# nemochina2008/soundgen_beta

Measured on AMD Instinct MI355X. Metric: synthesized audio samples/sec (whole node) @44.1 kHz; RMS error vs R ref, higher is better.
Workload: dtype fp32 (fp64 phase)

## Files before the change

### soundgen_beta_amd/csrc/sg_exec.cpp

```cpp
#include "sg_exec.h"
#include "sg_amp.h"
#include "sg_launch.h"
#include "sg_sine_check.h"
#include "sg_prof.h"

#include <algorithm>
#include <chrono>
#include <exception>
#include <thread>
#include <cmath>
#include <climits>
#include <atomic>
#include <map>
#include <cstdlib>
#include <cstdio>
#include <cstring>
#include <string>
#include <type_traits>

namespace sg {

static void split_finalize_tiles(Batch& B) {
  const int64_t copy_tile = SG_COPY_TILE;
  B.fin_tiles.clear();
  B.fin_tiles_hp.clear();
  B.copy_tiles.clear();
  for (const SgSylTile& t : B.syl_tiles) {
    const SgSyllable& sy = B.syls[t.syl];
    if (sy.hp) {
      B.fin_tiles_hp.push_back(t);
      continue;
    }
    const int64_t end = std::min<int64_t>(t.k0 + 1024, sy.L);
    const int pend = sy.piece0 + sy.npiece;
    bool ok = sy.env.kind == 0 && sy.drift.nk == 0 && sy.genv.kind == 0;
    for (int p = t.piece; ok && p < pend && B.pieces[p].start < end; ++p) ok = B.pieces[p].nterms <= 0;
    if (!ok) {
      B.fin_tiles.push_back(t);
      continue;
    }
    for (int p = t.piece; p < pend && B.pieces[p].start < end; ++p) {
      const SgPiece& pc = B.pieces[p];
      const int64_t a = std::max<int64_t>(t.k0, pc.start), b = std::min<int64_t>(end, pc.start + pc.len);
      if (b <= a) continue;
      SgCopyTile c{};
      const bool zero = pc.nterms == 0;
      c.src = zero ? 0 : pc.t[0].src + (a - pc.start);
      c.dst = sy.out_off + a;
      c.k0 = a;
      c.L = sy.L;
      c.n = (int32_t)(b - a);
      c.max_slot = sy.max_slot;
      c.fade = sy.fade;
      c.syl = t.syl;
      c.flags = (sy.dst_fs ? SG_COPY_FS : 0) | (zero ? SG_COPY_ZERO : 0) |
                (!zero && ((c.src - c.dst) & 3) == 0 ? SG_COPY_VEC : 0);
      if (!B.copy_tiles.empty()) {
        SgCopyTile& q = B.copy_tiles.back();
        if ((q.flags & SG_COPY_VEC) && (c.flags & SG_COPY_VEC) && q.syl == c.syl && q.flags == c.flags &&
            q.k0 + q.n == c.k0 && q.src + q.n == c.src && q.n + c.n <= copy_tile) {
          q.n += c.n;
          continue;
        }
      }
      B.copy_tiles.push_back(c);
    }
  }
}

static bool direct_on() {
  const char* e = std::getenv("SG_TAB_DIRECT");
  return !(e && e[0] == '0');
}

struct TabSpans {
  std::vector<SgTabJob> jobs;
  std::vector<uint8_t> in_tab;
  std::vector<uint8_t> direct_syl;
  int64_t tasks = 0, direct = 0;
  int64_t samples = 0, terms = 0;
};
struct ColumnReader {
  const Batch& B;
  std::vector<std::pair<int64_t, int32_t>> by_off;
  std::vector<double> lg;
  explicit ColumnReader(const Batch& b) : B(b) {
    for (size_t j = 0; j < B.ampjobs.size(); ++j) by_off.push_back({B.ampjobs[j].amp_off, (int32_t)j});
    std::sort(by_off.begin(), by_off.end());
    lg.resize((size_t)B.amp_lg_rows + 2);
    for (size_t k = 0; k < lg.size(); ++k) lg[k] = std::log2((double)(k + 1));
  }
  int logn_max = SG_TAB_LOGN_MAX;
  int logn(int64_t a_off, int32_t Rn) const {
    auto it = std::upper_bound(by_off.begin(), by_off.end(), std::make_pair(a_off, INT32_MAX));
    if (it == by_off.begin()) return 0;
    const SgAmpJob& J = B.ampjobs[(size_t)std::prev(it)->second];
    const int64_t rel = a_off - J.amp_off;
    if (J.Rp <= 0 || rel % J.Rp != 0 || rel / J.Rp >= J.G || Rn > J.Rp) return 0;
    const int g = (int)(rel / J.Rp);
    double s0 = 0, s4 = 0;
    for (int r = 0; r < Rn; ++r) {
      double a = 0;
      if (r < J.R) a = J.src_off >= 0 ? (double)B.ampsrc[(size_t)(J.src_off + (int64_t)g * J.Rp + r)]
                                      : (double)(float)amp_value(B.ampcols.data() + J.col0, J, lg.data(), g, r);
      const double k = r + 1.0;
      s0 += std::fabs(a);
      s4 += std::fabs(a) * k * k * k * k;
    }
    if (!(s0 > 0)) return 0;
    const double two_pi4 = 1558.5454565440389;
    for (int b = SG_TAB_LOGN_MIN; b <= logn_max; ++b) {
      const double n4 = std::ldexp(1.0, 4 * b);
      if (two_pi4 * s4 / (384.0 * n4) <= SG_TAB_TOL * s0) return b;
    }
    return 0;
  }
};
struct TaskBlock {
  int64_t o;
  const SgWTask* p;
  int64_t n;
};
static std::vector<TaskBlock> task_blocks(const Batch& B) {
  std::vector<TaskBlock> tb;
  bulk_each(B.tasks_x, B.tasks, [&](int64_t o, const SgWTask* p, int64_t n) { tb.push_back(TaskBlock{o, p, n}); });
  return tb;
}
template <class F>
static void for_blocks(size_t n, F&& f) {
  const size_t nt = std::min<size_t>(n, std::min(16u, std::max(1u, std::thread::hardware_concurrency())));
  if (nt <= 1) {
    for (size_t i = 0; i < n; ++i) f(i);
    return;
  }
  std::atomic<size_t> next{0};
  std::vector<std::exception_ptr> errs(nt);
  auto work = [&](size_t t) {
    try {
      for (size_t i; (i = next.fetch_add(1)) < n;) f(i);
    } catch (...) {
      errs[t] = std::current_exception();
    }
  };
  std::vector<std::thread> pool;
  for (size_t t = 1; t < nt; ++t) pool.emplace_back(work, t);
  work(0);
  for (auto& th : pool) th.join();
  for (auto& e : errs)
    if (e) std::rethrow_exception(e);
}
struct TabBlock {
  std::vector<SgTabJob> jobs;
  int64_t direct = 0, samples = 0, terms = 0;
};
static void group_block(const Batch& B, const ColumnReader& cols, const TaskBlock& blk, TabSpans& S, TabBlock& out) {
  auto tab_task = [](const SgWTask& t) {
    return t.flags == (SG_TASK_CONST | SG_TASK_LIN) && t.R <= SG_ROWS_F32 && t.Rn > 0;
  };
  auto direct_ok = [&](const SgWTask& t, int64_t r0, int64_t r1) {
    if (t.syl < 0 || t.syl >= (int32_t)B.syls.size() || !direct_on()) return false;
    const SgSyllable& sy = B.syls[(size_t)t.syl];
    if (sy.hp || sy.env.kind != 0 || sy.genv.kind != 0 || sy.drift.nk != 0 || sy.nptile != 0) return false;
    if (r0 != sy.task0 || r1 != sy.task0 + sy.ntask || r1 - r0 > SG_TAB_TASKS) return false;
    for (int32_t p = sy.piece0; p < sy.piece0 + sy.npiece; ++p)
      if (B.pieces[(size_t)p].nterms > 0) return false;
    return true;
  };
  const int per_job = SG_TAB_TASKS;
  int64_t run0 = -1, run_samples = 0;
  SgWTask first{};
  auto close_run = [&](int64_t end) {
    if (run0 < 0) return;
    const int logn = run_samples >= (int64_t(4) << SG_TAB_LOGN_MIN) ? cols.logn(first.a_off, first.Rn) : 0;
    if (logn && run_samples >= (int64_t(4) << logn)) {
      const bool dir = end - run0 <= per_job && direct_ok(first, run0, end);
      if (dir) {
        S.direct_syl[(size_t)first.syl] = 1;
        ++out.direct;
      }
      for (int64_t i = run0; i < end; i += per_job) {
        const int32_t n = (int32_t)std::min<int64_t>(per_job, end - i);
        out.jobs.push_back(SgTabJob{first.a_off, first.Rn, (int32_t)i, n, logn, first.syl, dir ? SG_TAB_DIRECT : 0});
        for (int64_t q = i; q < i + n; ++q) S.in_tab[(size_t)q] = 1;
      }
      out.samples += run_samples;
      out.terms += run_samples * first.Rn;
    }
    run0 = -1;
  };
  for (int64_t k = 0; k < blk.n; ++k) {
    const SgWTask& t = blk.p[k];
    const bool ok = tab_task(t);
    if (run0 >= 0 && !(ok && t.a_off == first.a_off && t.Rn == first.Rn && t.syl == first.syl)) close_run(blk.o + k);
    if (ok && run0 < 0) {
      run0 = blk.o + k;
      first = t;
      run_samples = 0;
    }
    if (ok) run_samples += t.len;
  }
  close_run(blk.o + blk.n);
}
struct TaskClasses {
  std::vector<int32_t> tlong, tshort, tall, tallp, thp;
  std::vector<int32_t> srun, trun;
};
static void run_start(std::vector<int32_t>& runs, const std::vector<int32_t>& list, int32_t& syl, const SgWTask& t) {
  const int32_t pos = (int32_t)list.size() - 1;
  if (runs.empty() || t.syl != syl || pos - runs.back() >= SG_RUN_TASKS) runs.push_back(pos);
  syl = t.syl;
}
static void classify_block(const TaskBlock& blk, const std::vector<uint8_t>& in_tab, TaskClasses& c) {
  int32_t ssyl = -1, tsyl = -1;
  for (int64_t k = 0; k < blk.n; ++k) {
    const SgWTask& t = blk.p[k];
    const int32_t i = (int32_t)(blk.o + k);
    const bool shrt = t.len <= 64 && !(t.flags & SG_TASK_ENV);
    if (!in_tab.empty() && in_tab[(size_t)i]) continue;
    if (t.flags & SG_TASK_HP) c.thp.push_back(i);
    else if (t.R > SG_ROWS_F32) {
      if (shrt) {
        c.tallp.push_back(i);
        run_start(c.trun, c.tallp, tsyl, t);
      } else {
        c.tall.push_back(i);
      }
    } else if (shrt) {
      c.tshort.push_back(i);
      run_start(c.srun, c.tshort, ssyl, t);
    } else {
      c.tlong.push_back(i);
    }
  }
}
static TabSpans group_tables(const Batch& B, bool tables, TaskClasses* classes) {
  TabSpans S;
  const std::vector<TaskBlock> tb = task_blocks(B);
  std::vector<TabBlock> tabs(tb.size());
  std::vector<TaskClasses> cls(classes ? tb.size() : 0);
  if (tables) {
    S.in_tab.assign((size_t)bulk_size(B.tasks_x, B.tasks), 0);
    S.direct_syl.assign(B.syls.size(), 0);
  }
  const ColumnReader cols(B);
  for_blocks(tb.size(), [&](size_t i) {
    if (tables) group_block(B, cols, tb[i], S, tabs[i]);
    if (classes) classify_block(tb[i], S.in_tab, cls[i]);
  });
  for (TabBlock& t : tabs) {
    S.jobs.insert(S.jobs.end(), t.jobs.begin(), t.jobs.end());
    S.direct += t.direct;
    S.samples += t.samples;
    S.terms += t.terms;
  }
  for (const SgTabJob& j : S.jobs) S.tasks += j.n;
  if (classes) {
    auto cat = [&](std::vector<int32_t> TaskClasses::*m) {
      std::vector<int32_t>& dst = classes->*m;
      dst.clear();
      size_t n = 0;
      for (const TaskClasses& c : cls) n += (c.*m).size();
      dst.reserve(n);
      for (const TaskClasses& c : cls) dst.insert(dst.end(), (c.*m).begin(), (c.*m).end());
    };
    auto runs = [&](std::vector<int32_t> TaskClasses::*r, std::vector<int32_t> TaskClasses::*m) {
      std::vector<int32_t>& dst = classes->*r;
      dst.clear();
      int32_t base = 0;
      for (const TaskClasses& c : cls) {
        for (int32_t x : c.*r) dst.push_back(base + x);
        base += (int32_t)(c.*m).size();
      }
      dst.push_back(base);
    };
    runs(&TaskClasses::srun, &TaskClasses::tshort);
    runs(&TaskClasses::trun, &TaskClasses::tallp);
    cat(&TaskClasses::tlong);
    cat(&TaskClasses::tshort);
    cat(&TaskClasses::tall);
    cat(&TaskClasses::tallp);
    cat(&TaskClasses::thp);
  }
  return S;
}

static void debug_plan_stats(const Batch& B) {
  std::fprintf(stderr, "sg plan: %zu sine tasks, %zu syllables, %zu copy tiles, %zu general finalize tiles\n",
               (size_t)bulk_size(B.tasks_x, B.tasks), B.syls.size(), B.copy_tiles.size(), B.fin_tiles.size());
  {
    double fry = 0, plain = 0;
    int64_t nfry = 0;
    for (const SgEpoch& e : B.epochs) {
      const double b = (double)(2 * e.G - 1) * e.R * 4;
      if (e.invD < 1) { fry += b; ++nfry; } else plain += b;
    }
    std::fprintf(stderr, "sg plan: amplitude bytes: plain epochs %.3g, subharmonic epochs %.3g (%lld of %zu)\n", plain,
                 fry, (long long)nfry, B.epochs.size());
  }
  {
    const TabSpans T = group_tables(B, true, nullptr);
    int64_t cl = 0, cl_samples = 0;
    bulk_each(B.tasks_x, B.tasks, [&](int64_t, const SgWTask* p, int64_t n) {
      for (int64_t k = 0; k < n; ++k)
        if (p[k].flags == (SG_TASK_CONST | SG_TASK_LIN)) { ++cl; cl_samples += p[k].len; }
    });
    int64_t hist[13] = {0};
    for (const SgTabJob& j : T.jobs) ++hist[j.logn];
    std::fprintf(stderr, "sg plan: wavetable jobs %zu, %lld direct syllables (N = 256/512/1024/2048: %lld %lld %lld %lld; %zu tasks, %lld samples, %.3g terms); CONST|LIN tasks %lld (%lld samples)\n",
                 T.jobs.size(), (long long)T.direct, (long long)hist[8], (long long)hist[9], (long long)hist[10], (long long)hist[11],
                 (size_t)T.tasks, (long long)T.samples, (double)T.terms, (long long)cl,
                 (long long)cl_samples);
  }
  {
    int64_t all = 0, ident = 0, ni = 0, ident_items = 0, noisy = 0, noisy_cov = 0, other = 0, env_only = 0, env_kind[4] = {0, 0, 0, 0};
    for (const SgMix& m : B.mixes[0]) {
      all += m.len;
      bool id = m.mult.kind == 0 && m.am_lo == 0 && m.to_fs == 1 && m.base_kind == SG_BASE_NONE;
      for (int32_t i = m.item0; i < m.item0 + m.nitems && id; ++i) {
        const SgNoiseItem& it = B.items[(size_t)i];
        id = it.ola < 0 && it.fade < 2 && it.strength.kind == 0 && !(it.flags & SG_ITEM_F64);
      }
      if (id) { ident += m.len; ident_items += m.nitems; }
      ni += m.nitems;
      if (!id && m.mult.kind == 0 && m.to_fs == 1) {
        std::vector<std::pair<int64_t, int64_t>> iv;
        for (int32_t i = m.item0; i < m.item0 + m.nitems; ++i) {
          const SgNoiseItem& it = B.items[(size_t)i];
          if (it.ola >= 0) iv.push_back({std::max<int64_t>(0, it.off), std::min(m.len, it.off + it.len)});
        }
        std::sort(iv.begin(), iv.end());
        int64_t cov = 0, e = 0;
        for (auto& q : iv) { const int64_t a0 = std::max(q.first, e); if (q.second > a0) cov += q.second - a0; e = std::max(e, q.second); }
        noisy += m.len;
        noisy_cov += cov;
      } else if (!id) {
        other += m.len;
        bool vo = m.to_fs == 1;
        for (int32_t i = m.item0; i < m.item0 + m.nitems && vo; ++i) vo = B.items[(size_t)i].ola < 0;
        if (vo && m.mult.kind != 0) { env_only += m.len; env_kind[m.mult.kind & 3]++; }
      }
    }
    std::fprintf(stderr, "sg plan: pre-filter mixes %zu, %lld samples; voiced-only %lld samples (%lld of %lld items)\n",
                 B.mixes[0].size(), (long long)all, (long long)ident, (long long)ident_items, (long long)ni);
    std::fprintf(stderr, "sg plan: pre-filter mixes with noise %lld samples (%lld under noise), enveloped or fp64 %lld "
                 "(voiced-only with the global envelope %lld; contour kinds 1/2/3: %lld %lld %lld)\n",
                 (long long)noisy, (long long)noisy_cov, (long long)other, (long long)env_only, (long long)env_kind[1],
                 (long long)env_kind[2], (long long)env_kind[3]);
  }
  {
    int64_t j1 = 0, jm = 0, cols = 0, bins = 0;
    for (const SgEnvJob& j : B.envjobs) {
      (j.nc == 1 ? j1 : jm)++;
      cols += j.nc;
      bins += (int64_t)j.nc * j.nr;
    }
    std::fprintf(stderr, "sg plan: envelope jobs %zu (%lld one-column), %lld columns, %lld bins, %zu wave tasks\n",
                 B.envjobs.size(), (long long)j1, (long long)cols, (long long)bins, B.envtasks.size());
  }
  std::vector<SgWTask> tasks;
  bulk_each(B.tasks_x, B.tasks, [&](int64_t, const SgWTask* p, int64_t n) { tasks.insert(tasks.end(), p, p + n); });
  double terms[2] = {0, 0};
  int64_t ntask[2] = {0, 0}, rmax = 0, samples[2] = {0, 0};
  std::map<int, int64_t> rh;
  int64_t nshort[2] = {0, 0}, lh[2][5] = {{0}};
  double sterms[2] = {0, 0};
  {
    int64_t nh = 0, sh = 0, lh64 = 0;
    double th = 0, rn = 0;
    for (const SgWTask& t : tasks)
      if (t.flags & SG_TASK_HP) {
        ++nh; sh += t.len; lh64 += t.len <= 64;
        th += (double)t.Rn * t.len * ((t.flags & SG_TASK_CONST) ? 1 : 2);
        rn += t.Rn;
      }
    std::fprintf(stderr, "sg plan: fp64 tasks %lld (%lld samples, %lld of <= 64 samples, %.3g chain terms, mean Rn %.1f)\n",
                 (long long)nh, (long long)sh, (long long)lh64, th, nh ? rn / nh : 0.0);
  }
  for (const SgWTask& t : tasks) {
    const int k = t.R > SG_ROWS_F32 ? 1 : 0;
    terms[k] += (double)t.R * t.len * ((t.flags & SG_TASK_CONST) ? 1 : 2);
    ++ntask[k];
    samples[k] += t.len;
    if (t.len <= 64) { ++nshort[k]; sterms[k] += (double)t.R * t.len * ((t.flags & SG_TASK_CONST) ? 1 : 2); }
    lh[k][t.len <= 64 ? 0 : t.len <= 128 ? 1 : t.len <= 256 ? 2 : t.len <= 512 ? 3 : 4]++;
    if (k) {
      rmax = std::max<int64_t>(rmax, t.R);
      rh[t.R < 256 ? 0 : t.R < 512 ? 1 : t.R < 1024 ? 2 : t.R < 2048 ? 3 : 4]++;
    }
  }
  std::fprintf(stderr, "sg plan: sine tasks fp32 %lld (%lld samples, %.3g chain terms), tall %lld (%lld samples, %.3g chain terms, max R %lld; R<256 %lld, <512 %lld, <1024 %lld, <2048 %lld, more %lld)\n",
               (long long)ntask[0], (long long)samples[0], terms[0], (long long)ntask[1], (long long)samples[1], terms[1],
               (long long)rmax, (long long)rh[0], (long long)rh[1], (long long)rh[2], (long long)rh[3], (long long)rh[4]);
  for (int k = 0; k < 2; ++k)
    std::fprintf(stderr, "sg plan: %s tasks <= 64 samples: %lld (%.3g chain terms); len <=64/128/256/512/more: %lld %lld %lld %lld %lld\n",
                 k ? "tall" : "fp32", (long long)nshort[k], sterms[k], (long long)lh[k][0], (long long)lh[k][1],
                 (long long)lh[k][2], (long long)lh[k][3], (long long)lh[k][4]);
}

void finalize_plan(Batch& B) {
  split_finalize_tiles(B);
  if (std::getenv("SG_DEBUG_PLAN")) debug_plan_stats(B);
  B.ptiles.clear();
  bool any_hp = false;
  for (int pass = 0; pass < 2; ++pass) {
    if (pass == 1) B.ptile_hp = (int64_t)B.ptiles.size();
    for (size_t s = 0; s < B.syls.size(); ++s) {
      SgSyllable& sy = B.syls[s];
      if ((sy.hp != 0) != (pass == 1)) continue;
      any_hp |= sy.hp != 0;
      sy.ptile0 = (int32_t)B.ptiles.size();
      for (int32_t p = sy.piece0; p < sy.piece0 + sy.npiece; ++p)
        if (B.pieces[p].nterms > 0)
          for (int64_t q0 = 0; q0 < B.pieces[p].len; q0 += 256) B.ptiles.push_back(SgSylTile{(int32_t)s, p, q0});
      sy.nptile = (int32_t)B.ptiles.size() - sy.ptile0;
    }
  }
  B.slices.clear();
  const int64_t nsyl = (int64_t)B.syls.size();
  if (nsyl == 0) return;
  int64_t total = 0;
  for (const SgSyllable& sy : B.syls) total += sy.L;
  int slices = SG_SLICES;
  if (any_hp) slices = 1;
  const int K = (int)std::min<int64_t>(slices, nsyl);
  int64_t acc = 0, ft = 0, ct = 0;
  int32_t s0 = 0;
  for (int32_t s = 0; s < nsyl; ++s) {
    acc += B.syls[s].L;
    const bool cut = s == nsyl - 1 || acc * K >= total * ((int64_t)B.slices.size() + 1);
    if (!cut) continue;
    Slice c{};
    c.s0 = s0; c.s1 = s + 1;
    c.t0 = B.syls[s0].task0;
    c.t1 = B.syls[s].task0 + B.syls[s].ntask;
    c.p0 = K == 1 ? 0 : B.syls[s0].ptile0;
    c.p1 = K == 1 ? B.ptile_hp : B.syls[s].ptile0 + B.syls[s].nptile;
    c.f0 = ft;
    while (ft < (int64_t)B.fin_tiles.size() && B.fin_tiles[ft].syl <= s) ++ft;
    c.f1 = ft;
    c.c0 = ct;
    while (ct < (int64_t)B.copy_tiles.size() && B.copy_tiles[ct].syl <= s) ++ct;
    c.c1 = ct;
    B.slices.push_back(c);
    s0 = s + 1;
  }
}

int64_t device_bytes(const Batch& B) { return (int64_t)arena_bytes(arena_counts(B)); }

void device_free(DevicePlan& D) {
  if (D.arena) (void)hipFree(D.arena);
  if (D.tabbuf) (void)hipFree(D.tabbuf);
  D.pcm.free();
// ... 384 lines not shown
```

### soundgen_beta_amd/csrc/sg_harm.hip

```cpp
#include <hip/hip_runtime.h>

#include "sg_dev.h"

#include "sg_amp.h"
#include "sg_devfn.h"

using sgd::contour_at;
using sgd::linear_at;
using sgd::wave_max;

constexpr int SG_LDS_ROWS = 256;



template <bool TWO>
__device__ __forceinline__ void stage_rows(float* __restrict__ la, float* __restrict__ ld, const float* __restrict__ A,
                                           const float* __restrict__ A1, int r0, int n, int lane) {
  for (int r = lane; r < n; r += 64) {
    const float a = A[r0 + r];
    la[r] = a;
    if (TWO) ld[r] = A1[r0 + r] - a;
  }
}

typedef float f2 __attribute__((ext_vector_type(2)));
__device__ __forceinline__ float vfma(float a, float b, float c) { return fmaf(a, b, c); }
__device__ __forceinline__ double vfma(double a, double b, double c) { return fma(a, b, c); }
__device__ __forceinline__ f2 vfma(f2 a, f2 b, f2 c) { return __builtin_elementwise_fma(a, b, c); }

#define SG_ROW(a, d)                                                  \
  {                                                                   \
    _Pragma("unroll") for (int s = 0; s < NS; ++s) {                  \
      const Acc av = TWO ? vfma(tt[s], (Acc)(d), (Acc)(a)) : (Acc)(a); \
      const Acc b = vfma(al[s], b1[s], av - b2[s]);                   \
      b2[s] = b1[s];                                                  \
      b1[s] = b;                                                      \
    }                                                                 \
  }
constexpr int SG_ROWS_IT = 8;
template <int NS, bool TWO, typename Acc>
__device__ __forceinline__ void clenshaw_lds(const float* __restrict__ la, const float* __restrict__ ld, int n,
                                             const Acc (&al)[NS], const Acc (&tt)[NS], Acc (&b1)[NS], Acc (&b2)[NS]) {
  const float4 z4 = make_float4(0.f, 0.f, 0.f, 0.f);
  if (n & 4) {
    const float4 A4 = *reinterpret_cast<const float4*>(la + n - 4);
    const float4 D4 = TWO ? *reinterpret_cast<const float4*>(ld + n - 4) : z4;
    SG_ROW(A4.w, D4.w)
    SG_ROW(A4.z, D4.z)
    SG_ROW(A4.y, D4.y)
    SG_ROW(A4.x, D4.x)
    n -= 4;
  }
#pragma unroll 1
  for (int r = n - SG_ROWS_IT; r >= 0; r -= SG_ROWS_IT) {
    const float4 A4 = *reinterpret_cast<const float4*>(la + r + 4);
    const float4 D4 = TWO ? *reinterpret_cast<const float4*>(ld + r + 4) : z4;
    const float4 A0 = *reinterpret_cast<const float4*>(la + r);
    const float4 D0 = TWO ? *reinterpret_cast<const float4*>(ld + r) : z4;
    SG_ROW(A4.w, D4.w)
    SG_ROW(A4.z, D4.z)
    SG_ROW(A4.y, D4.y)
    SG_ROW(A4.x, D4.x)
    SG_ROW(A0.w, D0.w)
    SG_ROW(A0.z, D0.z)
    SG_ROW(A0.y, D0.y)
    SG_ROW(A0.x, D0.x)
  }
}

template <bool TWO, bool LIN>
__device__ __forceinline__ void sample_setup(const SgWTask& T, int l, float& t, float& al, float& sn) {
  t = TWO ? fmaf((float)l, T.xby, T.tc0) * T.rdx : 0.f;
  const double m = (double)(T.mbase + l);
  const double P = LIN ? fma(m, T.c1, T.c0) : fma(m, fma(m, fma(m, fma(m, T.c4, T.c3), T.c2), T.c1), T.c0);
  const double v = P;
  const float x = (float)(v - rint(v));
  sn = __builtin_amdgcn_sinf(x);
  al = 2.f * __builtin_amdgcn_cosf(x);
}

template <int NS, bool TWO>
__device__ __forceinline__ void clenshaw_pk(const float* __restrict__ la, const float* __restrict__ ld, int n,
                                            const float (&al)[NS], const float (&tt)[NS], float (&b1)[NS],
                                            float (&b2)[NS]) {
  constexpr int NP = NS / 2;
  f2 al2[NP], t2[NP], p1[NP], p2[NP];
#pragma unroll
  for (int i = 0; i < NP; ++i) {
    al2[i] = f2{al[2 * i], al[2 * i + 1]};
    t2[i] = f2{tt[2 * i], tt[2 * i + 1]};
    p1[i] = f2{b1[2 * i], b1[2 * i + 1]};
    p2[i] = f2{b2[2 * i], b2[2 * i + 1]};
  }
  clenshaw_lds<NP, TWO, f2>(la, ld, n, al2, t2, p1, p2);
#pragma unroll
  for (int i = 0; i < NP; ++i) {
    b1[2 * i] = p1[i].x; b1[2 * i + 1] = p1[i].y;
    b2[2 * i] = p2[i].x; b2[2 * i + 1] = p2[i].y;
  }
}
template <int NS, bool TWO, typename Acc>
__device__ __forceinline__ void clenshaw_any(const float* __restrict__ la, const float* __restrict__ ld, int n,
                                             const Acc (&al)[NS], const Acc (&tt)[NS], Acc (&b1)[NS], Acc (&b2)[NS]) {
  if constexpr (sizeof(Acc) == 4 && NS % 2 == 0)
    clenshaw_pk<NS, TWO>(la, ld, n, al, tt, b1, b2);
  else
    clenshaw_lds<NS, TWO, Acc>(la, ld, n, al, tt, b1, b2);
}

template <bool TWO, bool LIN>
__device__ __forceinline__ void sample_setup(const SgWTask& T, int l, float& t, double& al, double& sn) {
  t = TWO ? fmaf((float)l, T.xby, T.tc0) * T.rdx : 0.f;
  const double m = (double)(T.mbase + l);
  const double P = LIN ? fma(m, T.c1, T.c0) : fma(m, fma(m, fma(m, fma(m, T.c4, T.c3), T.c2), T.c1), T.c0);
  double cs;
  sincospi(2.0 * (P - rint(P)), &sn, &cs);
  al = 2.0 * cs;
}

template <int NS, bool TWO, bool ENV, bool LIN, typename Acc, typename WT = float>
__device__ __forceinline__ void run_slots(const SgWTask& T, bool staged, float* __restrict__ la, float* __restrict__ ld,
                                          const float* __restrict__ amps, const SgSyllable* __restrict__ syls,
                                          const double* __restrict__ cknots, WT* __restrict__ W, int l0, int lane,
                                          float& tmax, const float (&rc)[8], const float (&rs)[8]) {
  constexpr bool ROT = LIN && sizeof(Acc) == 4 && NS > 1;
  float t[NS];
  Acc al[NS], sn[NS], b1[NS], b2[NS];
  int l[NS];
  bool valid[NS];
#pragma unroll
  for (int s = 0; s < NS; ++s) {
    l[s] = l0 + 64 * s + lane;
    valid[s] = l[s] < T.len;
    b1[s] = b2[s] = (Acc)0;
    if (ROT && s > 0) {
      t[s] = TWO ? fmaf((float)l[s], T.xby, T.tc0) * T.rdx : 0.f;
      const float h = 0.5f * (float)al[0], s2 = 2.f * (float)sn[0];
      al[s] = fmaf((float)al[0], rc[s], -s2 * rs[s]);
      sn[s] = fmaf((float)sn[0], rc[s], h * rs[s]);
    } else {
      sample_setup<TWO, LIN>(T, valid[s] ? l[s] : 0, t[s], al[s], sn[s]);
    }
  }
  Acc tt[NS];
#pragma unroll
  for (int s = 0; s < NS; ++s) tt[s] = (Acc)t[s];
  if (staged) {
    clenshaw_any<NS, TWO, Acc>(la, ld, T.Rn, al, tt, b1, b2);
  } else {
    for (int r0 = (T.Rn - 1) / SG_LDS_ROWS * SG_LDS_ROWS; r0 >= 0; r0 -= SG_LDS_ROWS) {
      const int n = T.Rn - r0 < SG_LDS_ROWS ? T.Rn - r0 : SG_LDS_ROWS;
      stage_rows<TWO>(la, ld, amps + T.a_off, amps + T.d_off, r0, n, lane);
      clenshaw_any<NS, TWO, Acc>(la, ld, n, al, tt, b1, b2);
    }
  }
  const int jp0 = T.j0 + l0;
  if (!ENV && l0 + 64 * NS <= T.len && jp0 >= T.dj0 && jp0 + 64 * NS <= T.dj1) {
    WT* __restrict__ wp = W + T.w_off + jp0 + lane;
// ... 135 lines not shown
}

template <bool TWO>
__device__ __forceinline__ void run_pair(const SgWTask& P, const SgWTask& Q, float* __restrict__ la,
                                         float* __restrict__ ld, const float* __restrict__ amps,
                                         float* __restrict__ W, int lane, float& mp, float& mq,
                                         ColCache* cc = nullptr) {
#ifdef SG_DIAG_PAIR_NOROWS
  const int R = 0;
#else
  const int R = P.Rn > Q.Rn ? P.Rn : Q.Rn;
#endif
  if (SG_RUN_CACHE && cc) {
    const bool pc = P.flags & SG_TASK_CONST, qc = Q.flags & SG_TASK_CONST;
    ColCache nc;
    const int hn = (P.R > 64 || Q.R > 64) ? 2 : 1;
#pragma unroll
    for (int h = 0; h < 2; ++h) {
      if (h >= hn) break;
      const int r = lane + 64 * h;
      auto load = [&](int64_t off, int rows) { return r < rows ? amps[off + r] : 0.f; };
      const float pa = P.a_off == cc->off ? cc->v[h] : load(P.a_off, P.R);
      const float pd = TWO && !pc ? (P.d_off == cc->off ? cc->v[h] : load(P.d_off, P.R)) : pa;
      const float qa = Q.a_off == P.a_off ? pa
                       : Q.a_off == P.d_off && TWO && !pc ? pd
                       : Q.a_off == cc->off ? cc->v[h] : load(Q.a_off, Q.R);
      const float qd = TWO && !qc ? (Q.d_off == P.d_off && !pc ? pd : load(Q.d_off, Q.R)) : qa;
      if (r < R) {
        *reinterpret_cast<float2*>(la + 2 * r) = make_float2(pa, qa);
        if (TWO) *reinterpret_cast<float2*>(ld + 2 * r) = make_float2(pc ? 0.f : pd - pa, qc ? 0.f : qd - qa);
      }
      nc.v[h] = TWO && !qc ? qd : qa;
    }
    nc.off = TWO && !qc ? Q.d_off : Q.a_off;
    *cc = nc;
  } else {
    stage_pair<TWO>(P, Q, amps, la, ld, 0, R, lane);
  }
  const bool vp = lane < P.len, vq = lane < Q.len;
  float tp, alp, snp, tq, alq, snq;
  sample_setup<TWO, false>(P, vp ? lane : 0, tp, alp, snp);
  sample_setup<TWO, false>(Q, vq ? lane : 0, tq, alq, snq);
  const f2 al{alp, alq}, tpq{tp, tq};
  f2 b1{0.f, 0.f}, b2{0.f, 0.f};
#define SG_PROW(a, d)                                   \
  {                                                     \
    const f2 av = TWO ? vfma(tpq, (d), (a)) : (a);      \
    const f2 b = vfma(al, b1, av - b2);                 \
    b2 = b1;                                            \
    b1 = b;                                             \
  }
  const float4 z4 = make_float4(0.f, 0.f, 0.f, 0.f);
#pragma unroll 1
  for (int r = R - 4; r >= 0; r -= 4) {
    const float4 A1 = *reinterpret_cast<const float4*>(la + 2 * r + 4);
    const float4 A0 = *reinterpret_cast<const float4*>(la + 2 * r);
    const float4 D1 = TWO ? *reinterpret_cast<const float4*>(ld + 2 * r + 4) : z4;
    const float4 D0 = TWO ? *reinterpret_cast<const float4*>(ld + 2 * r) : z4;
    SG_PROW((f2{A1.z, A1.w}), (f2{D1.z, D1.w}))
    SG_PROW((f2{A1.x, A1.y}), (f2{D1.x, D1.y}))
    SG_PROW((f2{A0.z, A0.w}), (f2{D0.z, D0.w}))
    SG_PROW((f2{A0.x, A0.y}), (f2{D0.x, D0.y}))
  }
#undef SG_PROW
  pair_store(P, Q, b1.x * snp, b1.y * snq, W, lane, mp, mq);
}

extern "C" __global__ __launch_bounds__(256) __attribute__((amdgpu_waves_per_eu(8))) void sg_sine_bank(
    const int32_t* __restrict__ idx, int64_t n, const SgWTask* __restrict__ tasks, const float* __restrict__ amps,
    const SgSyllable* __restrict__ syls, const double* __restrict__ cknots, float* __restrict__ W,
    float* __restrict__ taskmax) {
  __shared__ __attribute__((aligned(16))) float rows[4][2][SG_LDS_ROWS];
  const int lane = threadIdx.x & 63;
  const int wave = __builtin_amdgcn_readfirstlane(threadIdx.x >> 6);
  const int64_t k = (int64_t)sgd::xcd_swizzle(blockIdx.x, gridDim.x) * 4 + wave;
  if (k >= n) return;
  const int64_t ti = idx[k];
  const SgWTask T = tasks[ti];
  const float wm = wave_max(run_one(T, rows[wave][0], rows[wave][1], amps, syls, cknots, W, lane));
  if (lane == 0) taskmax[ti] = wm;
}

template <bool IDXPF, class PAIR>
__device__ __forceinline__ void run_of_pairs(const int32_t* __restrict__ idx, const int32_t* __restrict__ rs,
                                             int64_t nruns, const SgWTask* __restrict__ tasks,
                                             float* __restrict__ taskmax, PAIR&& pair) {
  const int lane = threadIdx.x & 63;
  const int wave = __builtin_amdgcn_readfirstlane(threadIdx.x >> 6);
  const int64_t r = (int64_t)sgd::xcd_swizzle(blockIdx.x, gridDim.x) * 4 + wave;
  if (r >= nruns) return;
  const int32_t k0 = rs[r], k1 = rs[r + 1];
  float m = -INFINITY;
  int32_t ip = idx[k0], iq = idx[k0 + 1 < k1 ? k0 + 1 : k0];
  for (int32_t k = k0; k < k1; k += 2) {
    if (!IDXPF) {
      ip = idx[k];
      iq = idx[k + 1 < k1 ? k + 1 : k];
    }
    const SgWTask P = tasks[ip];
    const SgWTask Q = tasks[iq];
    if (IDXPF && k + 2 < k1) {
      ip = idx[k + 2];
      iq = idx[k + 3 < k1 ? k + 3 : k + 2];
    }
    float mp, mq;
    pair(P, Q, wave, lane, mp, mq);
    m = fmaxf(m, fmaxf(mp, mq));
    __asm__ __volatile__("" ::: "memory");
  }
  m = wave_max(m);
  for (int32_t k = k0 + lane; k < k1; k += 64) taskmax[idx[k]] = k == k0 ? m : -INFINITY;
}

extern "C" __global__ __launch_bounds__(256) void sg_sine_bank_pairs(
    const int32_t* __restrict__ idx, const int32_t* __restrict__ rs, int64_t nruns,
    const SgWTask* __restrict__ tasks, const float* __restrict__ amps, float* __restrict__ W,
    float* __restrict__ taskmax) {
  __shared__ __attribute__((aligned(16))) float rows[4][2][SG_LDS_ROWS];
  ColCache cc;
  run_of_pairs<true>(idx, rs, nruns, tasks, taskmax,
               [&](const SgWTask& P, const SgWTask& Q, int wave, int lane, float& mp, float& mq) {
                 if ((P.flags & Q.flags) & SG_TASK_CONST) run_pair<false>(P, Q, rows[wave][0], rows[wave][1], amps, W, lane, mp, mq, &cc);
                 else run_pair<true>(P, Q, rows[wave][0], rows[wave][1], amps, W, lane, mp, mq, &cc);
               });
}


__device__ __forceinline__ void rs_setup(const SgWTask& T, int l, bool two, float& t, float& u, float& sg, float& sn) {
  t = two ? fmaf((float)l, T.xby, T.tc0) * T.rdx : 0.f;
  const double m = (double)(T.mbase + l);
  const double P = fma(m, fma(m, fma(m, fma(m, T.c4, T.c3), T.c2), T.c1), T.c0);
  const float x = (float)(P - rint(P));
  const float h = 3.14159265358979f * x;
  const float h2 = h * h;
  float s = fmaf(h2, 1.6059043836821614e-10f, -2.5052108385441720e-08f);
  s = fmaf(h2, s, 2.7557319223985893e-06f);
  s = fmaf(h2, s, -1.9841269841269841e-04f);
  s = fmaf(h2, s, 8.3333333333333333e-03f);
  s = fmaf(h2, s, -1.6666666666666667e-01f);
  s = fmaf(h2 * s, h, h);
  float c = fmaf(h2, -1.1470745597729725e-11f, 2.0876756987868099e-09f);
  c = fmaf(h2, c, -2.7557319223985891e-07f);
  c = fmaf(h2, c, 2.4801587301587302e-05f);
  c = fmaf(h2, c, -1.3888888888888889e-03f);
  c = fmaf(h2, c, 4.1666666666666667e-02f);
  c = fmaf(h2, c, -0.5f);
  c = fmaf(h2, c, 1.f);
  sn = 2.f * s * c;
  const bool pos = fabsf(x) <= 0.25f;
  sg = pos ? 1.f : -1.f;
  u = pos ? -4.f * s * s : 4.f * c * c;
}

template <bool TWO>
__device__ __forceinline__ void run_pair_rs(const SgWTask& P, const SgWTask& Q, float* __restrict__ la,
                                            float* __restrict__ ld, const float* __restrict__ amps,
                                            float* __restrict__ W, int lane, float& mp, float& mq) {
  const int R = P.Rn > Q.Rn ? P.Rn : Q.Rn;
  const bool vp = lane < P.len, vq = lane < Q.len;
  float tp, up, sgp, snp, tq, uq, sgq, snq;
  rs_setup(P, vp ? lane : 0, TWO, tp, up, sgp, snp);
  rs_setup(Q, vq ? lane : 0, TWO, tq, uq, sgq, snq);
  const f2 u{up, uq}, sg{sgp, sgq}, tpq{tp, tq};
  f2 b{0.f, 0.f}, d{0.f, 0.f};
#define SG_RPROW(a, dd)                                  \
  {                                                      \
    const f2 av = TWO ? vfma(tpq, (dd), (a)) : (a);      \
    f2 q = vfma(sg, d, av);                              \
    q = vfma(u, b, q);                                   \
    b = vfma(sg, b, q);                                  \
    d = q;                                               \
  }
  const float4 z4 = make_float4(0.f, 0.f, 0.f, 0.f);
  constexpr int CH = SG_LDS_ROWS / 2;
#pragma unroll 1
  for (int r0 = (R - 1) / CH * CH; r0 >= 0; r0 -= CH) {
    const int n = R - r0 < CH ? R - r0 : CH;
    stage_pair<TWO>(P, Q, amps, la, ld, r0, n, lane);
#pragma unroll 1
    for (int r = n - 4; r >= 0; r -= 4) {
      const float4 A1 = *reinterpret_cast<const float4*>(la + 2 * r + 4);
      const float4 A0 = *reinterpret_cast<const float4*>(la + 2 * r);
      const float4 D1 = TWO ? *reinterpret_cast<const float4*>(ld + 2 * r + 4) : z4;
      const float4 D0 = TWO ? *reinterpret_cast<const float4*>(ld + 2 * r) : z4;
      SG_RPROW((f2{A1.z, A1.w}), (f2{D1.z, D1.w}))
      SG_RPROW((f2{A1.x, A1.y}), (f2{D1.x, D1.y}))
      SG_RPROW((f2{A0.z, A0.w}), (f2{D0.z, D0.w}))
      SG_RPROW((f2{A0.x, A0.y}), (f2{D0.x, D0.y}))
    }
  }
#undef SG_RPROW
  pair_store(P, Q, b.x * snp, b.y * snq, W, lane, mp, mq);
}

__device__ __forceinline__ float run_one_tall(const SgWTask& T, float* __restrict__ la, float* __restrict__ ld,
                                              const float* __restrict__ amps, const SgSyllable* __restrict__ syls,
                                              const double* __restrict__ cknots, float* __restrict__ W, int lane) {
  if (T.flags & SG_TASK_ENV)
    return (T.flags & SG_TASK_CONST) ? run_task<false, true, false, double>(T, la, ld, amps, syls, cknots, W, lane)
                                     : run_task<true, true, false, double>(T, la, ld, amps, syls, cknots, W, lane);
  return (T.flags & SG_TASK_CONST) ? run_task<false, false, false, double>(T, la, ld, amps, syls, cknots, W, lane)
                                   : run_task<true, false, false, double>(T, la, ld, amps, syls, cknots, W, lane);
}

extern "C" __global__ __launch_bounds__(256) void sg_sine_bank_tall(
    const int32_t* __restrict__ idx, int64_t n, const SgWTask* __restrict__ tasks, const float* __restrict__ amps,
    const SgSyllable* __restrict__ syls, const double* __restrict__ cknots, float* __restrict__ W,
    float* __restrict__ taskmax) {
  __shared__ __attribute__((aligned(16))) float rows[4][2][SG_LDS_ROWS];
  const int lane = threadIdx.x & 63;
  const int wave = __builtin_amdgcn_readfirstlane(threadIdx.x >> 6);
  const int64_t k = (int64_t)sgd::xcd_swizzle(blockIdx.x, gridDim.x) * 4 + wave;
  if (k >= n) return;
  const int64_t ti = idx[k];
  const SgWTask T = tasks[ti];
  const float wm = wave_max(run_one_tall(T, rows[wave][0], rows[wave][1], amps, syls, cknots, W, lane));
  if (lane == 0) taskmax[ti] = wm;
}

extern "C" __global__ __launch_bounds__(256) void sg_sine_bank_tall_pairs(
    const int32_t* __restrict__ idx, const int32_t* __restrict__ rs, int64_t nruns,
    const SgWTask* __restrict__ tasks, const float* __restrict__ amps, float* __restrict__ W,
    float* __restrict__ taskmax) {
  __shared__ __attribute__((aligned(16))) float rows[4][2][SG_LDS_ROWS];
  run_of_pairs<false>(idx, rs, nruns, tasks, taskmax,
               [&](const SgWTask& P, const SgWTask& Q, int wave, int lane, float& mp, float& mq) {
                 if ((P.flags & Q.flags) & SG_TASK_CONST) run_pair_rs<false>(P, Q, rows[wave][0], rows[wave][1], amps, W, lane, mp, mq);
                 else run_pair_rs<true>(P, Q, rows[wave][0], rows[wave][1], amps, W, lane, mp, mq);
               });
}

__device__ __forceinline__ float run_one_hp(const SgWTask& T, float* __restrict__ la, float* __restrict__ ld,
                                            const float* __restrict__ amps, const SgSyllable* __restrict__ syls,
                                            const double* __restrict__ cknots, double* __restrict__ W, int lane) {
  const bool c = T.flags & SG_TASK_CONST;
  if (T.flags & SG_TASK_ENV)
    return c ? run_task<false, true, false, double, double>(T, la, ld, amps, syls, cknots, W, lane)
             : run_task<true, true, false, double, double>(T, la, ld, amps, syls, cknots, W, lane);
  if (T.flags & SG_TASK_LIN)
    return c ? run_task<false, false, true, double, double>(T, la, ld, amps, syls, cknots, W, lane)
             : run_task<true, false, true, double, double>(T, la, ld, amps, syls, cknots, W, lane);
  return c ? run_task<false, false, false, double, double>(T, la, ld, amps, syls, cknots, W, lane)
           : run_task<true, false, false, double, double>(T, la, ld, amps, syls, cknots, W, lane);
}

extern "C" __global__ __launch_bounds__(256) void sg_sine_bank_hp(
    const int32_t* __restrict__ idx, int64_t n, const SgWTask* __restrict__ tasks, const float* __restrict__ amps,
    const SgSyllable* __restrict__ syls, const double* __restrict__ cknots, double* __restrict__ W64,
    float* __restrict__ taskmax) {
  __shared__ __attribute__((aligned(16))) float rows[4][2][SG_LDS_ROWS];
  const int lane = threadIdx.x & 63;
  const int wave = __builtin_amdgcn_readfirstlane(threadIdx.x >> 6);
  const int64_t k = (int64_t)sgd::xcd_swizzle(blockIdx.x, gridDim.x) * 4 + wave;
  if (k >= n) return;
  const int64_t ti = idx[k];
  const SgWTask T = tasks[ti];
  const float wm = wave_max(run_one_hp(T, rows[wave][0], rows[wave][1], amps, syls, cknots, W64, lane));
  if (lane == 0) taskmax[ti] = wm;
}

template <typename V = float>
__device__ __forceinline__ V fade_at(int lf, int64_t L, int64_t k) {
  V f = 1;
  const V by = (V)1 / (V)(lf - 1);
  if (k < lf) f *= (k == lf - 1) ? (V)1 : (V)k * by;
  const int64_t kb = L - 1 - k;
  if (kb < lf) f *= (kb == lf - 1) ? (V)1 : (V)kb * by;
  return f;
}

constexpr int SG_TAB_THREADS = 512;
__device__ __forceinline__ void tab_build(float4* __restrict__ lt, const float* __restrict__ la, int Rn, int logn) {
  const int N = 1 << logn;
  float2* X = reinterpret_cast<float2*>(lt);
  float2* Y = X + N;
  float2* tw = X + 2 * N;
  const float pin = 3.14159265358979f / (float)N;
  for (int t = threadIdx.x; t < N / 4; t += SG_TAB_THREADS) {
    float sv, cv;
    sincospif(2.f * (float)t / (float)N, &sv, &cv);
    tw[t] = make_float2(cv, sv);
  }
  for (int m = threadIdx.x; m < N; m += SG_TAB_THREADS) {
    float z = 0.f;
    if (m >= 1 && m <= Rn) z = la[m - 1] * ((float)m * pin - 0.5f);
    else if (m >= N - Rn) z = la[N - m - 1] * ((float)(N - m) * pin + 0.5f);
    X[m] = make_float2(0.f, z);
  }
  __syncthreads();
  int Ns = 1;
  if (logn & 1) {
    for (int j = threadIdx.x; j < N / 2; j += SG_TAB_THREADS) {
      const float2 a = X[j], b = X[j + N / 2];
      Y[2 * j] = make_float2(a.x + b.x, a.y + b.y);
      Y[2 * j + 1] = make_float2(a.x - b.x, a.y - b.y);
    }
    __syncthreads();
    float2* t = X;
    X = Y;
    Y = t;
    Ns = 2;
  }
  auto cmul = [](float2 a, float2 b) { return make_float2(a.x * b.x - a.y * b.y, a.x * b.y + a.y * b.x); };
  for (; Ns < N; Ns <<= 2) {
    const int sh = logn - 2 - __builtin_ctz(Ns);
    for (int j = threadIdx.x; j < N / 4; j += SG_TAB_THREADS) {
      const int k = j & (Ns - 1);
      const float2 w1 = tw[k << sh], w2 = cmul(w1, w1), w3 = cmul(w2, w1);
      const float2 v0 = X[j], v1 = cmul(X[j + N / 4], w1), v2 = cmul(X[j + N / 2], w2),
                   v3 = cmul(X[j + 3 * N / 4], w3);
      const float2 s02 = make_float2(v0.x + v2.x, v0.y + v2.y), d02 = make_float2(v0.x - v2.x, v0.y - v2.y);
      const float2 s13 = make_float2(v1.x + v3.x, v1.y + v3.y), d13 = make_float2(v1.x - v3.x, v1.y - v3.y);
      const int o = (j - k) * 4 + k;
      Y[o] = make_float2(s02.x + s13.x, s02.y + s13.y);
      Y[o + Ns] = make_float2(d02.x - d13.y, d02.y + d13.x);
      Y[o + 2 * Ns] = make_float2(s02.x - s13.x, s02.y - s13.y);
      Y[o + 3 * Ns] = make_float2(d02.x + d13.y, d02.y - d13.x);
    }
    __syncthreads();
    float2* t = X;
    X = Y;
    Y = t;
  }
  constexpr int QM = (1 << SG_TAB_LOGN_MAX) / SG_TAB_THREADS;
  float4 c[QM];
#pragma unroll
  for (int q = 0; q < QM; ++q) {
    const int k = threadIdx.x + q * SG_TAB_THREADS;
    if (k < N) {
      const float2 p0 = X[k], p1 = X[(k + 1) & (N - 1)];
      c[q] = make_float4(p0.x, p0.y, 3.f * (p1.x - p0.x) - 2.f * p0.y - p1.y, 2.f * (p0.x - p1.x) + p0.y + p1.y);
    }
  }
  __syncthreads();
#pragma unroll
  for (int q = 0; q < QM; ++q) {
    const int k = threadIdx.x + q * SG_TAB_THREADS;
    if (k < N) lt[k] = c[q];
  }
}

struct TabTask;
template <int NB, bool FULL, typename TT>
__device__ __forceinline__ void tab_blocks(const float4* __restrict__ lt, int logn, const TT& T,
                                           float* __restrict__ w, uint32_t x, uint32_t dx, int l, float& tmax) {
  float4 c[NB];
  uint32_t xs[NB];
#pragma unroll
  for (int s = 0; s < NB; ++s) {
    xs[s] = x + (uint32_t)s * dx;
    c[s] = lt[xs[s] >> (32 - logn)];
  }
#pragma unroll
  for (int s = 0; s < NB; ++s) {
    const float f = (float)(xs[s] << logn) * 2.3283064365386963e-10f;
    const float y = fmaf(f, fmaf(f, fmaf(f, c[s].w, c[s].z), c[s].y), c[s].x);
    if (FULL) {
      w[64 * s] = y;
      tmax = fmaxf(tmax, y);
    } else if (l + 64 * s < T.len) {
      w[64 * s] = y;
      const int j = T.j0 + l + 64 * s;
      tmax = (j >= T.dj0 && j < T.dj1) ? fmaxf(tmax, y) : tmax;
    }
  }
}

struct TabTask {
  double c0, c1;
  int64_t off;
  int32_t mbase, j0, len, dj0, dj1, dk0;
};
template <bool STORE, bool CHECK>
__device__ __forceinline__ void tab_dblocks(const float4* __restrict__ lt, int logn, float* __restrict__ w,
                                            uint32_t x, uint32_t dx, int l, int ls, int le, float inv, int lf,
                                            int64_t L, int64_t k, float& tmax) {
  float4 c[4];
  uint32_t xs[4];
#pragma unroll
  for (int s = 0; s < 4; ++s) {
    xs[s] = x + (uint32_t)s * dx;
    c[s] = lt[xs[s] >> (32 - logn)];
// ... 508 lines not shown
```

Before: 14.02 billion.

## Pack short tall tasks into 16/32/64-lane slots within runs of pairs

Replaces the one-pair-per-step execution of short tall tasks with a packing scheme. Each run of up to 8 tasks is sorted by length and assigned 16/32/64-lane slots, so several short tasks share one wavefront step. Descriptors are staged in LDS, amplitude rows are staged per sub-block, and per-step max Rn, block count and flags are computed with LDS atomics. The aim is fewer recurrence steps and row trips and less idle lane work. In exchange it adds setup overhead, extra LDS, and padding to the maximum Rn of all tasks in a step. The plan debug output also prints packing statistics.

```diff
diff --git a/soundgen_beta_amd/csrc/sg_exec.cpp b/soundgen_beta_amd/csrc/sg_exec.cpp
--- a/soundgen_beta_amd/csrc/sg_exec.cpp
+++ b/soundgen_beta_amd/csrc/sg_exec.cpp
@@ -1,6 +1,7 @@
 #include "sg_exec.h"
 #include "sg_amp.h"
 #include "sg_launch.h"
+#include "sg_pack.h"
 #include "sg_sine_check.h"
 #include "sg_prof.h"
 
@@ -298,7 +299,51 @@
                  fry, (long long)nfry, B.epochs.size());
   }
   {
-    const TabSpans T = group_tables(B, true, nullptr);
+    TaskClasses C;
+    const TabSpans T = group_tables(B, true, &C);
+    {
+      std::vector<SgWTask> all;
+      bulk_each(B.tasks_x, B.tasks, [&](int64_t, const SgWTask* p, int64_t n) { all.insert(all.end(), p, p + n); });
+      auto stats = [&](const char* name, const std::vector<int32_t>& list, const std::vector<int32_t>& runs) {
+        int64_t hist[8] = {0}, steps0 = 0, steps1 = 0, trips0 = 0, trips1 = 0, samples = 0, slots = 0;
+        double rn = 0, used = 0, paid0 = 0, paid1 = 0;
+        for (size_t r = 0; r + 1 < runs.size(); ++r) {
+          const int n = runs[r + 1] - runs[r];
+          int len[SG_RUN_TASKS], start[SG_RUN_TASKS], Rs[SG_PACK_MAX_STEPS] = {0}, total = 0;
+          for (int i = 0; i < n; ++i) len[i] = all[(size_t)list[(size_t)(runs[r] + i)]].len;
+          for (int i = 0; i < n; ++i) {
+            const SgWTask& t = all[(size_t)list[(size_t)(runs[r] + i)]];
+            start[i] = sg_pack_start(len, n, i, &total);
+            Rs[start[i] / SG_PACK_SLOTS] = std::max(Rs[start[i] / SG_PACK_SLOTS], t.Rn);
+            ++hist[(t.len - 1) / 8];
+            samples += t.len;
+            slots += sg_pack_width(t.len);
+            rn += t.Rn;
+            used += (double)t.Rn * t.len;
+            if (i % 2 == 0) {
+              const int R = std::max(t.Rn, i + 1 < n ? all[(size_t)list[(size_t)(runs[r] + i + 1)]].Rn : 0);
+              ++steps0;
+              trips0 += R;
+              paid0 += 128.0 * R;
+            }
+          }
+          steps1 += sg_pack_steps(total);
+          for (int s = 0; s < sg_pack_steps(total); ++s) { trips1 += Rs[s]; paid1 += 128.0 * Rs[s]; }
+        }
+        const double nt = (double)std::max<size_t>(1, list.size());
+        std::fprintf(stderr, "sg plan: %s: %zu tasks in %zu runs, mean Rn %.1f; len <=8/16/../64: %lld %lld %lld %lld %lld %lld %lld %lld\n",
+                     name, list.size(), runs.empty() ? (size_t)0 : runs.size() - 1, rn / nt, (long long)hist[0],
+                     (long long)hist[1], (long long)hist[2], (long long)hist[3], (long long)hist[4], (long long)hist[5],
+                     (long long)hist[6], (long long)hist[7]);
+        std::fprintf(stderr, "sg plan: %s: steps %lld -> %lld (%.2f), row trips %lld -> %lld (%.2f); samples / lane slots %.2f; "
+                     "(row, sample) work used / paid %.3g / %.3g = %.2f -> / %.3g = %.2f\n",
+                     name, (long long)steps0, (long long)steps1, steps0 ? (double)steps1 / steps0 : 0.0, (long long)trips0,
+                     (long long)trips1, trips0 ? (double)trips1 / trips0 : 0.0, slots ? (double)samples / slots : 0.0, used,
+                     paid0, paid0 > 0 ? used / paid0 : 0.0, paid1, paid1 > 0 ? used / paid1 : 0.0);
+      };
+      stats("short fp32 tasks (sg_sine_bank_pairs)", C.tshort, C.srun);
+      stats("short tall tasks (sg_sine_bank_tall_pairs)", C.tallp, C.trun);
+    }
     int64_t cl = 0, cl_samples = 0;
     bulk_each(B.tasks_x, B.tasks, [&](int64_t, const SgWTask* p, int64_t n) {
       for (int64_t k = 0; k < n; ++k)
diff --git a/soundgen_beta_amd/csrc/sg_harm.hip b/soundgen_beta_amd/csrc/sg_harm.hip
--- a/soundgen_beta_amd/csrc/sg_harm.hip
+++ b/soundgen_beta_amd/csrc/sg_harm.hip
@@ -4,6 +4,7 @@
 
 #include "sg_amp.h"
 #include "sg_devfn.h"
+#include "sg_pack.h"
 
 using sgd::contour_at;
 using sgd::linear_at;
@@ -445,15 +446,120 @@
   u = pos ? -4.f * s * s : 4.f * c * c;
 }
 
-template <bool TWO>
-__device__ __forceinline__ void run_pair_rs(const SgWTask& P, const SgWTask& Q, float* __restrict__ la,
-                                            float* __restrict__ ld, const float* __restrict__ amps,
-                                            float* __restrict__ W, int lane, float& mp, float& mq) {
-  const int R = P.Rn > Q.Rn ? P.Rn : Q.Rn;
-  const bool vp = lane < P.len, vq = lane < Q.len;
+constexpr int SG_DESC_STRIDE = 144;
+static_assert(SG_RUN_TASKS == 8 && sizeof(SgWTask) == 128, "64 lanes load 8 descriptors, 16 B each");
+static_assert(offsetof(SgWTask, len) == 104, "pack_run takes len from piece 6");
+template <int ROWS>
+struct PackLds {
+  static constexpr int BLK = 2 * ROWS + 4;
+  char desc[SG_RUN_TASKS * SG_DESC_STRIDE];
+  float la[4 * BLK], ld[4 * BLK];
+  int len[SG_RUN_TASKS];
+  int map[8 * SG_PACK_MAX_STEPS];
+  int R[SG_PACK_MAX_STEPS], nb[SG_PACK_MAX_STEPS], fl[SG_PACK_MAX_STEPS];
+};
+__device__ __forceinline__ void wave_sync() { __asm__ __volatile__("" ::: "memory"); }
+
+template <class PL>
+__device__ __forceinline__ int pack_run(PL& L, const int32_t* __restrict__ idx, const SgWTask* __restrict__ tasks,
+                                        int32_t k0, int n, int lane) {
+  const int t = lane >> 3, piece = lane & 7;
+  const int32_t ti = idx[k0 + (t < n ? t : n - 1)];
+  const int4 v = reinterpret_cast<const int4*>(tasks + ti)[piece];
+  *reinterpret_cast<int4*>(L.desc + t * SG_DESC_STRIDE + 16 * piece) = v;
+  if (piece == 6) L.len[t] = v.z;
+  if (lane < 8 * SG_PACK_MAX_STEPS) L.map[lane] = 8;
+  if (lane < SG_PACK_MAX_STEPS) {
+    L.R[lane] = 0;
+    L.nb[lane] = 1;
+    L.fl[lane] = SG_TASK_CONST;
+  }
+  wave_sync();
+  int total = 0;
+  const int start = sg_pack_start(L.len, n, lane < n ? lane : 0, &total);
+  if (lane < n) {
+    char* d = L.desc + lane * SG_DESC_STRIDE;
+    const SgWTask* T = reinterpret_cast<const SgWTask*>(d);
+    const int w = sg_pack_width(T->len), Rn = T->Rn, flags = T->flags;
+    *reinterpret_cast<int*>(d + 128) = start;
+    for (int q = 0; q < (w >> 4); ++q) L.map[(start >> 4) + q] = lane;
+    const int s = start >> 7;
+    static_assert(SG_PACK_SLOTS == 128, "step of a start slot");
+    atomicMax(&L.R[s], Rn);
+    atomicMax(&L.nb[s], w == 16 ? 4 : w == 32 ? 2 : 1);
+    atomicAnd(&L.fl[s], flags);
+  }
+  wave_sync();
+  return __builtin_amdgcn_readfirstlane(sg_pack_steps(total));
+}
+
+template <bool TWO, class PL>
+__device__ __forceinline__ void pack_stage(PL& L, int s, int r0, int n, int nb, const float* __restrict__ amps,
+                                           int lane) {
+  const int lg = nb >> 1;
+  const int b = lane & (nb - 1);
+  const int q = b << (2 - lg);
+  const int ep = L.map[8 * s + q], eq = L.map[8 * s + 4 + q];
+  const SgWTask* P = reinterpret_cast<const SgWTask*>(L.desc + (ep & 7) * SG_DESC_STRIDE);
+  const SgWTask* Q = reinterpret_cast<const SgWTask*>(L.desc + (eq & 7) * SG_DESC_STRIDE);
+  const int pRn = P->Rn, qRn = Q->Rn;
+  const bool pc = P->flags & SG_TASK_CONST, qc = Q->flags & SG_TASK_CONST;
+  const float* __restrict__ pa = amps + P->a_off;
+  const float* __restrict__ qa = amps + Q->a_off;
+  const float* __restrict__ pd = amps + (pc ? P->a_off : P->d_off);
+  const float* __restrict__ qd = amps + (qc ? Q->a_off : Q->d_off);
+  const int lp = pRn > 0 ? pRn - 1 : 0, lq = qRn > 0 ? qRn - 1 : 0;
+  const int np = (ep & 8) ? 0 : pRn, nq = (eq & 8) ? 0 : qRn;
+  float* __restrict__ la = L.la + b * PL::BLK;
+  float* __restrict__ ld = L.ld + b * PL::BLK;
+  for (int i0 = 0; i0 < (n << lg); i0 += 64) {
+    const int r = (i0 + lane) >> lg;
+    if (r >= n) break;
+    const int rr = r0 + r;
+    const int ip = rr < pRn ? rr : lp, iq = rr < qRn ? rr : lq;
+    const float ap0 = pa[ip], aq0 = qa[iq];
+    const float dp0 = TWO ? pd[ip] : 0.f, dq0 = TWO ? qd[iq] : 0.f;
+    const bool inp = rr < np, inq = rr < nq;
+    const float ap = inp ? ap0 : 0.f, aq = inq ? aq0 : 0.f;
+    *reinterpret_cast<float2*>(la + 2 * r) = make_float2(ap, aq);
+    if (TWO)
+      *reinterpret_cast<float2*>(ld + 2 * r) = make_float2(inp && !pc ? dp0 - ap : 0.f, inq && !qc ? dq0 - aq : 0.f);
+  }
+}
+
+template <class PL>
+__device__ __forceinline__ void pack_lane(const PL& L, int e, int lane, SgWTask& T, int& l, bool& valid, bool& live) {
+  const char* d = L.desc + (e & 7) * SG_DESC_STRIDE;
+  T = *reinterpret_cast<const SgWTask*>(d);
+  live = !(e & 8);
+  l = lane - (*reinterpret_cast<const int*>(d + 128) & 63);
+  valid = live && l < T.len;
+  if (!valid) l = 0;
+}
+
+__device__ __forceinline__ float pack_store(const SgWTask& T, int l, bool valid, bool live, float y,
+                                            float* __restrict__ W) {
+  if (valid) W[T.w_off + T.j0 + l] = y;
+  const int j = T.j0 + l;
+  return !live ? -INFINITY : valid && j >= T.dj0 && j < T.dj1 ? y : 0.f;
+}
+
+template <bool TWO, class PL>
+__device__ __forceinline__ float pack_step_rs(PL& L, int s, int R, int nb, const float* __restrict__ amps,
+                                              float* __restrict__ W, int lane) {
+  SgWTask P, Q;
+  int lp, lq;
+  bool vp, vq, livep, liveq;
+  pack_lane(L, L.map[8 * s + (lane >> 4)], lane, P, lp, vp, livep);
+  pack_lane(L, L.map[8 * s + 4 + (lane >> 4)], lane, Q, lq, vq, liveq);
   float tp, up, sgp, snp, tq, uq, sgq, snq;
-  rs_setup(P, vp ? lane : 0, TWO, tp, up, sgp, snp);
-  rs_setup(Q, vq ? lane : 0, TWO, tq, uq, sgq, snq);
+  rs_setup(P, lp, TWO, tp, up, sgp, snp);
+  rs_setup(Q, lq, TWO, tq, uq, sgq, snq);
+  if (P.flags & SG_TASK_CONST) tp = 0.f;
+  if (Q.flags & SG_TASK_CONST) tq = 0.f;
+  const int blk = lane >> (6 - (nb >> 1));
+  const float* __restrict__ la = L.la + blk * PL::BLK;
+  const float* __restrict__ ld = L.ld + blk * PL::BLK;
   const f2 u{up, uq}, sg{sgp, sgq}, tpq{tp, tq};
   f2 b{0.f, 0.f}, d{0.f, 0.f};
 #define SG_RPROW(a, dd)                                  \
@@ -469,7 +575,9 @@
 #pragma unroll 1
   for (int r0 = (R - 1) / CH * CH; r0 >= 0; r0 -= CH) {
     const int n = R - r0 < CH ? R - r0 : CH;
-    stage_pair<TWO>(P, Q, amps, la, ld, r0, n, lane);
+    wave_sync();
+    pack_stage<TWO>(L, s, r0, n, nb, amps, lane);
+    wave_sync();
 #pragma unroll 1
     for (int r = n - 4; r >= 0; r -= 4) {
       const float4 A1 = *reinterpret_cast<const float4*>(la + 2 * r + 4);
@@ -483,7 +591,32 @@
     }
   }
 #undef SG_RPROW
-  pair_store(P, Q, b.x * snp, b.y * snq, W, lane, mp, mq);
+  const float mp = pack_store(P, lp, vp, livep, b.x * snp, W), mq = pack_store(Q, lq, vq, liveq, b.y * snq, W);
+  return fmaxf(mp, mq);
+}
+
+template <class PL, class STEP>
+__device__ __forceinline__ void run_packed(PL (&lds)[4], const int32_t* __restrict__ idx,
+                                           const int32_t* __restrict__ rs, int64_t nruns,
+                                           const SgWTask* __restrict__ tasks, float* __restrict__ taskmax,
+                                           STEP&& step) {
+  const int lane = threadIdx.x & 63;
+  const int wave = __builtin_amdgcn_readfirstlane(threadIdx.x >> 6);
+  const int64_t r = (int64_t)sgd::xcd_swizzle(blockIdx.x, gridDim.x) * 4 + wave;
+  if (r >= nruns) return;
+  const int32_t k0 = rs[r], k1 = rs[r + 1];
+  if (k1 <= k0) return;
+  PL& L = lds[wave];
+  const int steps = pack_run(L, idx, tasks, k0, k1 - k0, lane);
+  float m = -INFINITY;
+  for (int s = 0; s < steps; ++s) {
+    const int R = __builtin_amdgcn_readfirstlane(L.R[s]), nb = __builtin_amdgcn_readfirstlane(L.nb[s]);
+    const bool two = !(__builtin_amdgcn_readfirstlane(L.fl[s]) & SG_TASK_CONST);
+    m = fmaxf(m, step(L, s, R, nb, two, lane));
+    wave_sync();
+  }
+  m = wave_max(m);
+  for (int32_t k = k0 + lane; k < k1; k += 64) taskmax[idx[k]] = k == k0 ? m : -INFINITY;
 }
 
 __device__ __forceinline__ float run_one_tall(const SgWTask& T, float* __restrict__ la, float* __restrict__ ld,
@@ -515,12 +648,11 @@
     const int32_t* __restrict__ idx, const int32_t* __restrict__ rs, int64_t nruns,
     const SgWTask* __restrict__ tasks, const float* __restrict__ amps, float* __restrict__ W,
     float* __restrict__ taskmax) {
-  __shared__ __attribute__((aligned(16))) float rows[4][2][SG_LDS_ROWS];
-  run_of_pairs<false>(idx, rs, nruns, tasks, taskmax,
-               [&](const SgWTask& P, const SgWTask& Q, int wave, int lane, float& mp, float& mq) {
-                 if ((P.flags & Q.flags) & SG_TASK_CONST) run_pair_rs<false>(P, Q, rows[wave][0], rows[wave][1], amps, W, lane, mp, mq);
-                 else run_pair_rs<true>(P, Q, rows[wave][0], rows[wave][1], amps, W, lane, mp, mq);
-               });
+  __shared__ __attribute__((aligned(16))) PackLds<SG_LDS_ROWS / 2> lds[4];
+  run_packed(lds, idx, rs, nruns, tasks, taskmax,
+             [&](PackLds<SG_LDS_ROWS / 2>& L, int s, int R, int nb, bool two, int lane) {
+               return two ? pack_step_rs<true>(L, s, R, nb, amps, W, lane) : pack_step_rs<false>(L, s, R, nb, amps, W, lane);
+             });
 }
 
 __device__ __forceinline__ float run_one_hp(const SgWTask& T, float* __restrict__ la, float* __restrict__ ld,
diff --git a/soundgen_beta_amd/csrc/sg_pack.h b/soundgen_beta_amd/csrc/sg_pack.h
--- /dev/null
+++ b/soundgen_beta_amd/csrc/sg_pack.h
@@ -0,0 +1,26 @@
+#pragma once
+
+#ifdef __HIP__
+#define SG_PACK_FN __attribute__((host)) __attribute__((device)) inline
+#else
+#define SG_PACK_FN inline
+#endif
+
+constexpr int SG_PACK_SLOTS = 128;
+constexpr int SG_PACK_MAX_STEPS = 4;
+
+SG_PACK_FN int sg_pack_width(int len) { return len <= 16 ? 16 : len <= 32 ? 32 : 64; }
+
+SG_PACK_FN int sg_pack_start(const int* len, int n, int i, int* total) {
+  int start = 0, sum = 0;
+  for (int j = 0; j < n; ++j) {
+    const int w = sg_pack_width(len[j]);
+    const bool before = len[j] > len[i] || (len[j] == len[i] && j < i);
+    start += before ? w : 0;
+    sum += w;
+  }
+  *total = sum;
+  return start;
+}
+
+SG_PACK_FN int sg_pack_steps(int total) { return (total + SG_PACK_SLOTS - 1) / SG_PACK_SLOTS; }
```

Measured after the change: 13.81 billion. -1.5%, worse.
